# poja/Cattus

Hardware: AMD Instinct MI355X
Metric: MCTS node-evals/sec (chess 20x256 net, batch 256) (higher is better)
Workload: dtype f16x2

## Files before the change

### cattus_amd/csrc/evaluator.hip

```cpp
#include <hip/hip_runtime.h>

#include <algorithm>
#include <atomic>
#include <chrono>
#include <condition_variable>
#include <cmath>
#include <cstdarg>
#include <cstdio>
#include <cstdlib>
#include <cstring>
#include <deque>
#include <functional>
#include <map>
#include <memory>
#include <mutex>
#include <new>
#include <shared_mutex>
#include <string>
#include <thread>
#include <vector>

#include <dlfcn.h>

#include "../../include/cattus_hip.h"
// ... 102 lines not shown
    void* p = nullptr;
    bool owned = true;
    ~DevBuf() {
        if (p && owned) (void)hipFree(p);
    }
    int alloc(size_t bytes, DevArena* arena = nullptr) {
        if (p && owned) (void)hipFree(p);
        p = nullptr, owned = true;
        if (arena && (p = arena->take(bytes ? bytes : 16))) {
            owned = false;
            return CATTUS_OK;
        }
        hipError_t e = hipMalloc(&p, bytes ? bytes : 16);
        if (e != hipSuccess) return fail(CATTUS_E_NOMEM, "hipMalloc(%zu) failed: %s", bytes, hipGetErrorString(e));
        return CATTUS_OK;
    }
    int upload(const void* src, size_t bytes, DevArena* arena = nullptr) {
        int rc = alloc(bytes, arena);
        if (rc) return rc;
        HIP_TRY(hipMemcpy(p, src, bytes, hipMemcpyHostToDevice));
        return CATTUS_OK;
    }
    template <typename T>
    T* as() const {
        return reinterpret_cast<T*>(p);
    }
};

struct PinnedBuf {
    void* p = nullptr;
    ~PinnedBuf() {
        if (p) (void)hipHostFree(p);
    }
    int alloc(size_t bytes) {
        hipError_t e = hipHostMalloc(&p, bytes ? bytes : 16, hipHostMallocDefault);
        if (e != hipSuccess) return fail(CATTUS_E_NOMEM, "hipHostMalloc(%zu) failed: %s", bytes, hipGetErrorString(e));
        return CATTUS_OK;
    }
    template <typename T>
    T* as() const {
        return reinterpret_cast<T*>(p);
    }
};

std::shared_mutex g_pin_mu;
std::map<const char*, size_t> g_pinned;
struct Roctx {
    int (*push)(const char*) = nullptr;
    int (*pop)() = nullptr;
    Roctx() {
        const char* on = getenv("CATTUS_ROCTX");
        if (!on || on[0] != '1') return;
        for (const char* name : {"librocprofiler-sdk-roctx.so", "libroctx64.so"}) {
            if (void* h = dlopen(name, RTLD_NOW | RTLD_GLOBAL)) {
                push = reinterpret_cast<int (*)(const char*)>(dlsym(h, "roctxRangePushA"));
                pop = reinterpret_cast<int (*)()>(dlsym(h, "roctxRangePop"));
                if (push && pop) return;
                push = nullptr, pop = nullptr;
            }
        }
    }
};
const Roctx& roctx() {
    static const Roctx r;
    return r;
}
struct RoctxRange {
    bool on;
// ... 17 lines not shown
    return (const char*)p < it->first + it->second;
}

struct ConvLayer {
    DevBuf w, b;
    DevBuf wf;
    DevBuf wu, bw;
    uint32_t cin = 0;
};

struct ServerBatch {
    uint64_t seq = 0;
    uint32_t count = 0, collected = 0;
    bool sealed = false, running = false, done = false;
    int status = CATTUS_OK;
    std::string error;
    std::chrono::steady_clock::time_point t0;
    std::vector<uint64_t> planes;
    std::vector<float> policy, value;
    std::vector<uint8_t> taken;
};

constexpr int NLANES = CATTUS_HIP_LANES;

struct Lane {
    hipStream_t stream = nullptr;
    hipEvent_t done = nullptr;
    DevBuf d_planes, x0, a, t, y, hv, h1, d_policy, d_value;
    DevBuf d_legal_idx, d_legal_cnt, d_probs;
    uint32_t legal_stride = 0;
    PinnedBuf h_planes, h_policy, h_value;
    DevBuf tower_layers, tower_ready;
    PinnedBuf h_tower_err;
    uint32_t tower_nlayers = 0;
    std::mutex mu;
    ~Lane() {
        if (done) (void)hipEventDestroy(done);
        if (stream) (void)hipStreamDestroy(stream);
    }
};

}

struct cattus_eval {
    DevArena arena;
    cattus_net_desc d{};
    cattus_eval_config cfg{};
    bool tuned = false;
    bool simple = false;
    DevBuf d1w, d1b, d2w, d2b, svw, svb, spw, spb;
    bool wait_spin = true;
    Act act = Act::F32;
    uint32_t hw = 0, bpad = 0, cpad0 = 0;
    uint32_t slots = 64;
    uint32_t fpad = 0;
    bool tower64 = false;
    bool resident_tower = true;
    DevBuf t64_layers;
    bool tower64s = false;
    DevBuf t64s_bias;
    bool t64s_fuse_heads = true;
    int t64s_depth = 0;
    bool pack_separately = false;
    int t64_force_ch = 0;
    bool winograd = false;
    bool wino_k4 = true;
    bool wino_k8 = false;
    bool wino_persist = true;
    std::atomic<bool> persist_ok{true};
    uint32_t persist_spin = 1u << 18;
    uint32_t cus = 0;
    bool wino_inplace = true;
    bool split_wfrag = true;
    bool stream_shift_on = true;
    int stream_shift = 0;
    ConvOpts conv_opts;
    DevBuf d_saturated;
    bool t64_layer_steps = true;
    int device = 0;

    ConvLayer stem;
    std::vector<std::unique_ptr<ConvLayer>> c1, c2;
    DevBuf head_w, head_b, w1t, b1, w2, b2, wpt, bp;
    uint32_t kvp = 0, kpp = 0;

    Lane lanes[NLANES];
    std::atomic<unsigned> lane_rr{0};

    std::mutex stat_mu;
    cattus_stats stats{};
    uint64_t stats_tower_fallbacks = 0;

    std::mutex srv_mu;
    std::condition_variable srv_cv, done_cv;
    std::deque<std::unique_ptr<ServerBatch>> batches;
    uint64_t next_seq = 1;
    bool flush_req = false, stop = false;
    std::thread servers[NLANES];

    ~cattus_eval() {
        {
            std::lock_guard<std::mutex> lk(srv_mu);
            stop = true;
        }
        srv_cv.notify_all();
        done_cv.notify_all();
        for (auto& t : servers)
            if (t.joinable()) t.join();
    }
};

namespace {

size_t blob_floats(const cattus_net_desc& d) {
    const size_t hw = (size_t)d.board * d.board, F = d.filters;
    if (F == 0) {
        const size_t K = (size_t)d.planes * hw;
        return 2 * (K * K + K) + K + 1 + (size_t)d.moves * K + d.moves;
    }
    size_t n = F * d.planes * 9 + 4 * F;
    n += (size_t)d.blocks * (2 * F * F * 9 + 6 * F);
    n += (size_t)d.vhc * F + 2 * (size_t)d.vhc + (size_t)FC_HIDDEN * d.vhc * hw + FC_HIDDEN + FC_HIDDEN + 1;
    n += (size_t)d.phc * F + 2 * (size_t)d.phc + (size_t)d.moves * d.phc * hw + d.moves;
    return n;
}

bool wino_shape_ok(const cattus_eval* e, uint32_t cin, uint32_t cout) {
    return e->wino_k4 ? wino4_supported(e->bpad, cin, cout, e->d.board) : wino_supported(e->bpad, cin, cout, e->d.board);
}

std::mutex g_chain_mu;
hipEvent_t g_chain[64] = {};
int chain_persistent_launch(int device, hipStream_t st, const std::function<void()>& launch) {
    std::lock_guard<std::mutex> lk(g_chain_mu);
    hipEvent_t& ev = g_chain[device & 63];
    if (!ev) {
        HIP_TRY(hipEventCreateWithFlags(&ev, hipEventDisableTiming));
    } else {
        HIP_TRY(hipStreamWaitEvent(st, ev, 0));
    }
    launch();
    HIP_TRY(hipEventRecord(ev, st));
    return CATTUS_OK;
}

int upload_conv(cattus_eval* e, ConvLayer& L, const Folded& f, uint32_t cout, uint32_t cin, uint32_t cout_pad, uint32_t cin_pad) {
    int rc;
    if (!e->tuned) {
        L.cin = cin;
        if ((rc = L.b.upload(f.b.data(), cout * sizeof(float)))) return rc;
        return L.w.upload(f.w.data(), f.w.size() * sizeof(float));
    }
    L.cin = cin_pad;
    if (e->act == Act::F16S) {
        std::vector<float> b((size_t)2 * cout_pad, 0.0f);
        memcpy(b.data(), f.b.data(), cout * sizeof(float));
        std::vector<_Float16> w((size_t)9 * cout_pad * 2 * cin_pad, (_Float16)0.0f);
        for (uint32_t co = 0; co < cout_pad; co++) {
            float m = 0.0f;
            if (co < cout)
                for (uint32_t t = 0; t < 9; t++)
                    for (uint32_t ci = 0; ci < cin; ci++) m = std::max(m, fabsf(f.w[((size_t)t * cout + co) * cin + ci]));
            int sh = 0;
            if (m > 0.0f && std::isfinite(m)) sh = std::min(100, std::max(-100, 10 - ilogbf(m)));
            b[cout_pad + co] = ldexpf(1.0f, -sh);
            if (co >= cout) continue;
            for (uint32_t t = 0; t < 9; t++)
                for (uint32_t ci = 0; ci < cin; ci++) {
                    const float ws = ldexpf(f.w[((size_t)t * cout + co) * cin + ci], sh);
                    const _Float16 hi = (_Float16)ws;
                    const _Float16 lo = (_Float16)(ws - (float)hi);
                    _Float16* row = &w[((size_t)t * cout_pad + co) * 2 * cin_pad + (size_t)(ci >> 5) * 64 + (ci & 31)];
                    row[0] = hi, row[32] = lo;
                }
// ... 253 lines not shown
    }

    const size_t bp_ = e->bpad, B = e->cfg.max_batch;
    const size_t esz = e->tuned ? (act_f16_family(e->act) ? 4 : (size_t)act_bytes(e->act)) : 4;
    const size_t hesz = e->tuned ? (size_t)act_bytes(head_act(e->act)) : 4;
    const size_t slots = e->tuned ? e->slots : hw;
    const size_t FA = e->tuned ? FP : F;
    for (Lane& L : e->lanes) {
        HIP_TRY(hipStreamCreateWithFlags(&L.stream, hipStreamNonBlocking));
        HIP_TRY(hipEventCreateWithFlags(&L.done, hipEventBlockingSync | hipEventDisableTiming));
        if ((rc = L.d_planes.alloc(B * d.planes * e->cfg.plane_words * 8))) return rc;
        if ((rc = L.x0.alloc(bp_ * slots * e->cpad0 * esz))) return rc;
        if ((rc = L.a.alloc(bp_ * slots * FA * esz, &e->arena))) return rc;
        if ((rc = L.t.alloc(bp_ * slots * FA * esz, &e->arena))) return rc;
        if ((rc = L.y.alloc(bp_ * slots * FA * esz, e->wino_inplace ? nullptr : &e->arena))) return rc;
        const size_t hv_bytes = (size_t)(e->tuned ? (bp_ + 31) / 32 * 32 : bp_) * (e->kvp + e->kpp) * hesz;
        if ((rc = L.hv.alloc(hv_bytes))) return rc;
        HIP_TRY(hipMemset(L.hv.p, 0, hv_bytes));
        if ((rc = L.h1.alloc(bp_ * FC_HIDDEN * 4))) return rc;
        if ((rc = L.d_policy.alloc(B * d.moves * 4))) return rc;
        if ((rc = L.d_value.alloc(B * 4))) return rc;
        if ((rc = L.h_planes.alloc(B * d.planes * e->cfg.plane_words * 8))) return rc;
        if ((rc = L.h_policy.alloc(B * d.moves * 4))) return rc;
        if ((rc = L.h_value.alloc(B * 4))) return rc;
        if (e->tuned && e->act == Act::F16S && e->wino_k4 && e->wino_persist && e->wino_inplace && d.blocks > 0 && e->c1[0]->wu.p) {
            std::vector<Wino4TowerLayer> tl;
            for (uint32_t i = 0; i < d.blocks; i++) {
                tl.push_back(Wino4TowerLayer{L.a.as<float>(), e->c1[i]->wu.p, e->c1[i]->bw.as<float>(), nullptr, L.t.as<float>()});
                tl.push_back(Wino4TowerLayer{L.t.as<float>(), e->c2[i]->wu.p, e->c2[i]->bw.as<float>(), L.a.as<float>(), L.a.as<float>()});
            }
            L.tower_nlayers = (uint32_t)tl.size();
            if ((rc = L.tower_layers.upload(tl.data(), tl.size() * sizeof(Wino4TowerLayer)))) return rc;
            if ((rc = L.tower_ready.alloc(64 + (size_t)tl.size() * (bp_ / 4) * 4))) return rc;
            if ((rc = L.h_tower_err.alloc(4))) return rc;
            *L.h_tower_err.as<unsigned>() = 0;
        }
    }
    return CATTUS_OK;
}

struct TowerTimer {
    std::vector<hipEvent_t> ev;
    size_t used = 0;
};

int enqueue_forward(cattus_eval* e, Lane& L, const uint64_t* d_planes, uint32_t n, float* d_policy, float* d_value,
                    hipStream_t st, TowerTimer* tt = nullptr) {
    const cattus_net_desc& d = e->d;
    const uint32_t F = d.filters, hw = e->hw, S = d.board, w64 = e->cfg.plane_words;
    auto ev = [&](bool stop) -> hipEvent_t {
        if (!tt || tt->used >= tt->ev.size()) return nullptr;
        (void)stop;
        return tt->ev[tt->used++];
    };
    void *a = L.a.p, *t = L.t.p, *y = L.y.p;
    uint32_t nb = n;
    if (e->simple) {
        const uint32_t K = d.planes * hw;
        launch_planes_to_tensor_nchw(d_planes, n, d.planes, w64, S, n, L.x0.as<float>(), st);
        launch_dense(L.x0.as<float>(), K, e->d1w.as<float>(), e->d1b.as<float>(), n, K, K, (float*)a, 1, st);
        launch_dense((float*)a, K, e->d2w.as<float>(), e->d2b.as<float>(), n, K, K, (float*)t, 1, st);
        launch_dense((float*)t, K, e->svw.as<float>(), e->svb.as<float>(), n, K, 1, d_value, 2, st);
        launch_dense((float*)t, K, e->spw.as<float>(), e->spb.as<float>(), n, K, d.moves, d_policy, 0, st);
        hipError_t serr = hipGetLastError();
        if (serr != hipSuccess) return fail(CATTUS_E_DEVICE, "kernel launch failed: %s", hipGetErrorString(serr));
        return CATTUS_OK;
    }
    if (e->tuned) {
// ... 17 lines not shown
            ta.bias_all = e->t64s_bias.as<float>();
            ta.n = n, ta.C = d.planes, ta.w64 = w64, ta.S = S, ta.nlayers = 1 + 2 * d.blocks;
            if (e->t64s_fuse_heads) {
                ta.head_w = e->head_w.as<float>(), ta.head_b = e->head_b.as<float>(), ta.hv = L.hv.as<float>();
                ta.hv_pol = (uint32_t)((e->bpad + 31) / 32 * 32) * e->kvp, ta.kvp = e->kvp, ta.kpp = e->kpp, ta.vhc = d.vhc, ta.ocn = d.vhc + d.phc;
            } else {
                ta.out = (float*)a;
            }
            hipEvent_t s0 = ev(false), s1 = ev(true);
            launch_tower64_split(ta, nb * e->slots, e->t64s_depth, st, s0, s1);
        } else {
            const bool fused_stem = d.planes <= 32 && e->cpad0 == (uint32_t)act_kc(e->act) && !e->pack_separately;
            const StemInput stem_in{d_planes, n, d.planes, w64};
            if (!fused_stem) launch_pack_planes_nhwc(e->act, d_planes, n, nb, d.planes, w64, S, e->cpad0, L.x0.p, st);
            hipEvent_t s0 = ev(false), s1 = ev(true);
            const int last_flags = act_f16_family(e->act) ? CONV_OUT_F32 : 0;
            const bool wfrag = e->act == Act::F16S && e->split_wfrag;
            const int wflag = wfrag ? CONV_W_FRAG : 0;
            auto wptr = [&](const ConvLayer& c) { return wfrag ? c.wf.p : c.w.p; };
            launch_conv3x3_mfma(e->act, L.x0.p, wptr(e->stem), e->stem.b.as<float>(), nullptr, a, nb, e->cpad0, FP, S, st, s0, s1,
                                fused_stem ? &stem_in : nullptr,
                                wflag | (d.blocks == 0 ? last_flags : e->act == Act::F16S && e->c1[0]->wu.p ? CONV_OUT_F32 | CONV_WINO_IN : 0), e->conv_opts);
            const bool wino = d.blocks > 0 && e->c1[0]->wu.p != nullptr;
            auto conv = [&](const ConvLayer& c, const void* in, const void* res, void* out, int lflags) {
                hipEvent_t s0 = ev(false), s1 = ev(true);
                if (wino && e->wino_k8) launch_conv3x3_wino8((const float*)in, c.wu.p, c.bw.as<float>(), (const float*)res, (float*)out, nb, FP, FP, st, s0, s1, e->conv_opts.saturated);
                else if (wino && e->wino_k4) launch_conv3x3_wino4((const float*)in, c.wu.p, c.bw.as<float>(), (const float*)res, (float*)out, nb, FP, FP, st, s0, s1, e->conv_opts.saturated);
                else if (wino) launch_conv3x3_wino((const float*)in, c.wu.p, c.bw.as<float>(), (const float*)res, (float*)out, nb, FP, FP, st, s0, s1, e->conv_opts.saturated);
                else launch_conv3x3_mfma(e->act, in, wptr(c), c.b.as<float>(), res, out, nb, FP, FP, S, st, s0, s1, nullptr, wflag | lflags, e->conv_opts);
            };
            if (wino && !e->wino_k8 && L.tower_nlayers && e->persist_ok.load(std::memory_order_relaxed) && wino4_tower_fits(nb, FP, e->cus)) {
                hipEvent_t s0 = ev(false), s1 = ev(true);
                unsigned* const tower_err = L.tower_ready.as<unsigned>();
                HIP_TRY(hipMemsetAsync(L.tower_ready.p, 0, 64 + (size_t)L.tower_nlayers * (nb / 4) * 4, st));
                int crc = chain_persistent_launch(e->device, st, [&] {
                    launch_tower_wino4(L.tower_layers.as<Wino4TowerLayer>(), L.tower_nlayers, tower_err + 16, tower_err,
                                       e->conv_opts.saturated, nb, FP, e->persist_spin, e->cus, st, s0, s1);
                });
                if (crc) return crc;
                HIP_TRY(hipMemcpyAsync(L.h_tower_err.p, tower_err, 4, hipMemcpyDeviceToHost, st));
            } else
            for (uint32_t i = 0; i < d.blocks; i++) {
                conv(*e->c1[i], a, nullptr, t, 0);
                if (wino && e->wino_inplace) {
                    conv(*e->c2[i], t, a, a, 0);
                    continue;
                }
                conv(*e->c2[i], t, a, y, i + 1 == d.blocks ? last_flags : 0);
                std::swap(a, y);
            }
        }
    } else {
        launch_planes_to_tensor_nchw(d_planes, n, d.planes, w64, S, n, L.x0.as<float>(), st);
        hipEvent_t s0 = ev(false), s1 = ev(true);
        launch_conv3x3_generic(L.x0.as<float>(), e->stem.w.as<float>(), e->stem.b.as<float>(), nullptr, (float*)a, n,
                               d.planes, F, S, st, s0, s1);
        for (uint32_t i = 0; i < d.blocks; i++) {
            s0 = ev(false), s1 = ev(true);
            launch_conv3x3_generic((float*)a, e->c1[i]->w.as<float>(), e->c1[i]->b.as<float>(), nullptr, (float*)t, n, F,
                                   F, S, st, s0, s1);
            s0 = ev(false), s1 = ev(true);
            launch_conv3x3_generic((float*)t, e->c2[i]->w.as<float>(), e->c2[i]->b.as<float>(), (float*)a, (float*)y, n,
                                   F, F, S, st, s0, s1);
            std::swap(a, y);
        }
    }
    const uint32_t kv = d.vhc * hw, kp = d.phc * hw;
    if (e->tuned) {
        HeadsMfma hd{};
        hd.conv_w = e->head_w.p, hd.conv_b = e->head_b.as<float>(), hd.hv = L.hv.p;
        hd.w1 = e->w1t.p, hd.b1 = e->b1.as<float>(), hd.h1 = L.h1.as<float>();
        hd.wp = e->wpt.p, hd.bp = e->bp.as<float>(), hd.policy = d_policy;
        hd.hw = hw, hd.vhc = d.vhc, hd.phc = d.phc, hd.kvp = e->kvp, hd.kpp = e->kpp, hd.M = d.moves;
// ... 62 lines not shown
    }
    const void* src_planes = planes;
    if (!direct) {
        memcpy(L.h_planes.p, planes, pbytes);
        src_planes = L.h_planes.p;
    }
    HIP_TRY(hipMemcpyAsync(L.d_planes.p, src_planes, pbytes, hipMemcpyHostToDevice, L.stream));
    auto copy_out = [&]() -> int {
        if (lg) {
            HIP_TRY(hipMemcpyAsync(L.d_legal_idx.p, lg->idx, (size_t)n * lg->stride * 2, hipMemcpyHostToDevice, L.stream));
            HIP_TRY(hipMemcpyAsync(L.d_legal_cnt.p, lg->cnt, (size_t)n * 2, hipMemcpyHostToDevice, L.stream));
            if (launch_legal_softmax(L.d_policy.as<float>(), d.moves, L.d_legal_idx.as<uint16_t>(), L.d_legal_cnt.as<uint16_t>(),
                                     lg->stride, n, L.d_probs.as<float>(), L.stream))
                return fail(CATTUS_E_INVALID, "legal stride %u exceeds 1024", lg->stride);
            HIP_TRY(hipMemcpyAsync(lg->probs, L.d_probs.p, (size_t)n * lg->stride * 4, hipMemcpyDeviceToHost, L.stream));
        } else {
            HIP_TRY(hipMemcpyAsync(direct ? (void*)policy : L.h_policy.p, L.d_policy.p, (size_t)n * d.moves * 4, hipMemcpyDeviceToHost, L.stream));
        }
        HIP_TRY(hipMemcpyAsync(direct ? (void*)value : L.h_value.p, L.d_value.p, (size_t)n * 4, hipMemcpyDeviceToHost, L.stream));
        return CATTUS_OK;
    };
    auto run_batch = [&]() -> int {
        int rc = enqueue_forward(e, L, L.d_planes.as<uint64_t>(), n, L.d_policy.as<float>(), L.d_value.as<float>(), L.stream);
        if (rc) return rc;
        if ((rc = copy_out())) return rc;
        if (e->wait_spin) {
            HIP_TRY(hipStreamSynchronize(L.stream));
        } else {
            HIP_TRY(hipEventRecord(L.done, L.stream));
            HIP_TRY(hipEventSynchronize(L.done));
        }
        return CATTUS_OK;
    };
    int rc = run_batch();
    if (rc) return rc;
    if (L.h_tower_err.p && *L.h_tower_err.as<volatile unsigned>() != 0) {
        *L.h_tower_err.as<volatile unsigned>() = 0;
        e->persist_ok.store(false, std::memory_order_relaxed);
        {
            std::lock_guard<std::mutex> sl(e->stat_mu);
            e->stats_tower_fallbacks += 1;
        }
        if ((rc = run_batch())) return rc;
    }
    if (!direct) {
        if (!lg) memcpy(policy, L.h_policy.p, (size_t)n * d.moves * 4);
        memcpy(value, L.h_value.p, (size_t)n * 4);
    }
    account(e, n, std::chrono::duration<double>(std::chrono::steady_clock::now() - t0).count());
    return CATTUS_OK;
}

ServerBatch* new_batch(cattus_eval* e) {
    auto b = std::make_unique<ServerBatch>();
    b->seq = e->next_seq++;
    b->planes.resize((size_t)e->cfg.max_batch * e->d.planes * e->cfg.plane_words);
    e->batches.push_back(std::move(b));
    return e->batches.back().get();
}

void server_loop(cattus_eval* e) {
    std::unique_lock<std::mutex> lk(e->srv_mu);
    for (;;) {
        ServerBatch* run = nullptr;
        for (auto& b : e->batches)
            if (b->sealed && !b->done && !b->running) {
                run = b.get();
                break;
            }
        if (!run && !e->batches.empty()) {
// ... 28 lines not shown
        run->error = err;
        run->done = true;
        e->done_cv.notify_all();
    }
}

}


CATTUS_API const char* cattus_hip_last_error(void) { return g_last_error.c_str(); }
CATTUS_API const char* cattus_hip_version(void) { return "cattus_hip 0.2 (gfx950)"; }
CATTUS_API const char* cattus_hip_runtime_note(void) { return g_runtime_note.c_str(); }

CATTUS_API const char* cattus_hip_tower_kernel(const cattus_eval* e) {
    if (!e) return "";
    if (e->simple) return "policy_fc_kernel";
    if (!e->tuned) return "conv3x3_generic_kernel";
    if (e->tower64) return "tower64_lds_kernel";
    if (e->tower64s) return "tower64_split_kernel";
    if (e->act == Act::F16S) return e->d.blocks > 0 && e->c1[0]->wu.p ? (e->wino_k8 ? "conv3x3_wino8_kernel" : e->wino_k4 ? (e->lanes[0].tower_nlayers && e->persist_ok.load() && wino4_tower_fits(e->bpad, e->fpad, e->cus) ? "tower_wino4_kernel" : "conv3x3_wino4_kernel") : "conv3x3_wino_kernel") : e->split_wfrag ? "conv3x3_splitw_kernel" : "conv3x3_split_kernel";
    return "conv3x3_mfma_v2_kernel";
}

CATTUS_API int cattus_hip_stream_shift(const cattus_eval* e) { return e ? e->stream_shift : 0; }

namespace {

struct Switches {
    std::map<std::string, std::string> kv;
    int parse(const char* text) {
        if (!text) return CATTUS_OK;
        static const char* const known[] = {"CATTUS_CONV_CB", "CATTUS_CONV_PBW", "CATTUS_FUSED_STEM", "CATTUS_T64_CH", "CATTUS_T64_LS", "CATTUS_SPLIT_W",
                                            "CATTUS_T64S_HEADS", "CATTUS_T64S_SHAPE", "CATTUS_TOWER64", "CATTUS_FORCE_GENERIC", "CATTUS_WINO_INPLACE",
                                            "CATTUS_ARENA", "CATTUS_WINO_KERNEL", "CATTUS_WINO_PERSIST", "CATTUS_WINO_SPIN", "CATTUS_STREAM_SHIFT"};
        const std::string s(text);
        size_t at = 0;
        while (at < s.size()) {
            size_t end = s.find(';', at);
            if (end == std::string::npos) end = s.size();
            const std::string item = s.substr(at, end - at);
            at = end + 1;
            if (item.empty()) continue;
            const size_t eq = item.find('=');
            if (eq == std::string::npos || eq == 0) return fail(CATTUS_E_INVALID, "diagnostic switch '%s' is not KEY=VALUE", item.c_str());
            const std::string key = item.substr(0, eq);
            bool ok = false;
            for (const char* k : known) ok = ok || key == k;
            if (!ok) return fail(CATTUS_E_INVALID, "unknown diagnostic switch '%s'", key.c_str());
            kv[key] = item.substr(eq + 1);
        }
        return CATTUS_OK;
    }
    const char* get(const char* key) const {
        auto it = kv.find(key);
        return it == kv.end() ? nullptr : it->second.c_str();
    }
};

int create_impl(const void* weights, size_t nbytes, const cattus_eval_config* cfg_in, const char* switches, cattus_eval** out) {
    if (!out) return fail(CATTUS_E_INVALID, "out is NULL");
    *out = nullptr;
    if (!weights || !cfg_in) return fail(CATTUS_E_INVALID, "weights/cfg is NULL");
    cattus_eval_config cfg_copy{};
    if (cfg_in->struct_size == offsetof(cattus_eval_config, tower_form)) memcpy(&cfg_copy, cfg_in, offsetof(cattus_eval_config, tower_form));
    else if (cfg_in->struct_size == sizeof(cattus_eval_config)) cfg_copy = *cfg_in;
    else return fail(CATTUS_E_INVALID, "cfg.struct_size mismatch");
    cfg_copy.struct_size = sizeof(cattus_eval_config);
// ... 84 lines not shown
             : cfg->dtype == CATTUS_DTYPE_F16X2 ? Act::F16S
             : cfg->dtype == CATTUS_DTYPE_F16 ? Act::F16
                                              : Act::F32;
    if (!e->tuned && e->act != Act::F32)
        return fail(CATTUS_E_UNSUPPORTED, "bf16 / f16 / f16x2 need the MFMA tower: value + policy head channels <= 32 (got %u + %u)", d.vhc, d.phc);
    if (act_f16_family(e->act)) {
        int src = e->d_saturated.alloc(sizeof(unsigned));
        if (src) return src;
        HIP_TRY(hipMemset(e->d_saturated.p, 0, sizeof(unsigned)));
        e->conv_opts.saturated = e->d_saturated.as<unsigned>();
    }
    if (act_f16_family(e->act)) {
        if (d.planes > 32) return fail(CATTUS_E_UNSUPPORTED, "f16x2 / f16 take at most 32 input planes (got %u)", d.planes);
        e->pack_separately = false;
    }
    e->slots = tower_slots(d.board);
    e->fpad = e->tuned ? (d.filters + COUT_PER_WG - 1) / COUT_PER_WG * COUT_PER_WG : d.filters;
    const uint32_t bpw = e->tuned ? ROWS_PER_WG / e->slots : 1;
    e->bpad = (cfg->max_batch + bpw - 1) / bpw * bpw;
    const char* inplace_env = sw.get("CATTUS_WINO_INPLACE");
    e->wino_inplace = !(inplace_env && inplace_env[0] == '0');
    const char* arena_env = sw.get("CATTUS_ARENA");
    {
        const char* wk = sw.get("CATTUS_WINO_KERNEL");
        if (wk && strcmp(wk, "k16") != 0 && strcmp(wk, "k4") != 0 && strcmp(wk, "k8") != 0) return fail(CATTUS_E_INVALID, "CATTUS_WINO_KERNEL is k16, k4 or k8");
        e->wino_k8 = wk && strcmp(wk, "k8") == 0;
        e->wino_k4 = wk ? strcmp(wk, "k4") == 0 || e->wino_k8 : wino4_supported(e->bpad, e->fpad, e->fpad, d.board);
    }
    {
        const char* wp = sw.get("CATTUS_WINO_PERSIST");
        e->wino_persist = !(wp && wp[0] == '0');
        const char* ws = sw.get("CATTUS_WINO_SPIN");
        if (ws) e->persist_spin = (uint32_t)std::max(1L, atol(ws));
        hipDeviceProp_t prop;
        HIP_TRY(hipGetDeviceProperties(&prop, cfg->device));
        e->cus = (uint32_t)prop.multiProcessorCount;
    }
    if (cfg->tower_form == CATTUS_TOWER_WINOGRAD && !(e->tuned && e->act == Act::F16S && d.blocks > 0 && wino_shape_ok(e.get(), e->fpad, e->fpad)))
        return fail(CATTUS_E_UNSUPPORTED, "tower_form WINOGRAD needs dtype f16x2, an 8x8 board, at least one residual block and a multiple of 64 filters");
    if (e->tuned && e->act == Act::F16S && e->winograd && d.blocks > 0 && wino_shape_ok(e.get(), e->fpad, e->fpad) &&
        !(arena_env && arena_env[0] == '0')) {
        auto page = [](size_t b) { return (b + 4095) & ~(size_t)4095; };
        const size_t FPz = e->fpad, u_bytes = page(((size_t)16 * FPz * FPz * 2 + (size_t)WINO_RING_STAGES * 1024) * 2);
        const size_t act_bytes_ = page((size_t)e->bpad * e->slots * FPz * 4);
        const size_t want = 2 * (size_t)d.blocks * u_bytes + (size_t)NLANES * (e->wino_inplace ? 2 : 3) * act_bytes_ + (1u << 20);
        void* base = nullptr;
        if (hipMalloc(&base, want) == hipSuccess) e->arena.base = (char*)base, e->arena.cap = want;
        else (void)hipGetLastError();
    }
    int rc = build(e.get(), reinterpret_cast<const float*>((const char*)weights + HEADER_BYTES));
    if (rc) return rc;
    HIP_TRY(hipDeviceSynchronize());
    {
        std::lock_guard<std::mutex> lk(e->srv_mu);
        new_batch(e.get());
    }
    for (auto& t : e->servers) t = std::thread(server_loop, e.get());
    *out = e.release();
    return CATTUS_OK;
}

}

CATTUS_API int cattus_hip_create(const void* weights, size_t nbytes, const cattus_eval_config* cfg, cattus_eval** out) {
    return create_impl(weights, nbytes, cfg, nullptr, out);
}
// ... 14 lines not shown
    if (!e || !planes || !policy || !value) return fail(CATTUS_E_INVALID, "NULL argument");
    if (n < 1 || n > e->cfg.max_batch) return fail(CATTUS_E_INVALID, "invalid sample len %u, 1..=%u", n, e->cfg.max_batch);
    return eval_host(e, planes, n, policy, value);
}

CATTUS_API int cattus_hip_eval_legal(cattus_eval* e, const uint64_t* planes, uint32_t n, const uint16_t* legal_idx,
                                     const uint16_t* legal_count, uint32_t legal_stride, float* probs, float* value) {
    if (!e || !planes || !legal_idx || !legal_count || !probs || !value) return fail(CATTUS_E_INVALID, "NULL argument");
    if (n < 1 || n > e->cfg.max_batch) return fail(CATTUS_E_INVALID, "invalid sample len %u, 1..=%u", n, e->cfg.max_batch);
    if (legal_stride < 1 || legal_stride > 1024) return fail(CATTUS_E_INVALID, "legal_stride %u outside 1..=1024", legal_stride);
    for (uint32_t i = 0; i < n; i++) {
        if (legal_count[i] > legal_stride) return fail(CATTUS_E_INVALID, "leaf %u: %u legal moves > stride %u", i, legal_count[i], legal_stride);
        for (uint32_t k = 0; k < legal_count[i]; k++)
            if (legal_idx[(size_t)i * legal_stride + k] >= e->d.moves)
                return fail(CATTUS_E_INVALID, "leaf %u: policy index %u >= %u", i, legal_idx[(size_t)i * legal_stride + k], e->d.moves);
    }
    const LegalArgs lg{legal_idx, legal_count, legal_stride, probs};
    return eval_host(e, planes, n, nullptr, value, &lg);
}

CATTUS_API int cattus_hip_eval_device(cattus_eval* e, const uint64_t* d_planes, uint32_t n, float* d_policy, float* d_value,
                                      void* stream) {
    return cattus_hip_eval_device_lane(e, 0, d_planes, n, d_policy, d_value, stream);
}

CATTUS_API int cattus_hip_eval_device_lane(cattus_eval* e, uint32_t lane, const uint64_t* d_planes, uint32_t n, float* d_policy,
                                           float* d_value, void* stream) {
    if (!e || !d_planes || !d_policy || !d_value) return fail(CATTUS_E_INVALID, "NULL argument");
    if (n < 1 || n > e->cfg.max_batch) return fail(CATTUS_E_INVALID, "invalid sample len %u, 1..=%u", n, e->cfg.max_batch);
    if (lane >= NLANES) return fail(CATTUS_E_INVALID, "lane %u out of range (%d lanes)", lane, NLANES);
    Lane& L = e->lanes[lane];
    std::lock_guard<std::mutex> lk(L.mu);
    HIP_TRY(hipSetDevice(e->device));
    if (L.h_tower_err.p && *L.h_tower_err.as<volatile unsigned>() != 0) {
        *L.h_tower_err.as<volatile unsigned>() = 0;
        e->persist_ok.store(false, std::memory_order_relaxed);
        return fail(CATTUS_E_DEVICE, "an earlier batch on lane %u ran the tower as one launch and a hand-off wait in it gave up (the device was shared): that batch's "
                                     "outputs are invalid; this evaluator uses the per-layer launches from now on", lane);
    }
    hipStream_t st = (hipStream_t)stream;
    int rc = enqueue_forward(e, L, d_planes, n, d_policy, d_value, st);
    if (rc) return rc;
    std::lock_guard<std::mutex> sl(e->stat_mu);
    e->stats.batches += 1;
    e->stats.positions += n;
    if (n == e->cfg.max_batch) e->stats.full_batches += 1;
    return CATTUS_OK;
}

CATTUS_API int cattus_hip_lane_stream(cattus_eval* e, uint32_t lane, void** stream) {
    if (!e || !stream) return fail(CATTUS_E_INVALID, "NULL argument");
    if (lane >= NLANES) return fail(CATTUS_E_INVALID, "lane %u out of range (%d lanes)", lane, NLANES);
    *stream = (void*)e->lanes[lane].stream;
    return CATTUS_OK;
}

CATTUS_API int cattus_hip_submit(cattus_eval* e, const uint64_t* planes_one, uint64_t* ticket) {
    if (!e || !planes_one || !ticket) return fail(CATTUS_E_INVALID, "NULL argument");
    const size_t words = (size_t)e->d.planes * e->cfg.plane_words;
    std::unique_lock<std::mutex> lk(e->srv_mu);
    if (e->stop) return fail(CATTUS_E_STATE, "evaluator is shutting down");
    ServerBatch* cur = e->batches.empty() ? nullptr : e->batches.back().get();
    if (!cur || cur->sealed) cur = new_batch(e);
    const uint32_t slot = cur->count++;
    if (slot == 0) cur->t0 = std::chrono::steady_clock::now();
    memcpy(cur->planes.data() + slot * words, planes_one, words * 8);
    *ticket = (cur->seq << 32) | slot;
    const bool full = cur->count == e->cfg.max_batch;
    if (full) {
        cur->sealed = true;
        new_batch(e);
// ... 207 lines not shown
```

### cattus_amd/csrc/kernels.h

```cpp
#pragma once
#include <hip/hip_runtime.h>
#include <stdint.h>

namespace cattus {

inline uint32_t tower_slots(uint32_t S) { return S <= 8 ? 64u : 128u; }
constexpr int ROWS_PER_WG = 256;
constexpr int COUT_PER_WG = 64;

enum class Act : int { F32 = 0, BF16 = 1, F16S = 2, F16 = 3 };

inline bool act_two_bytes(Act a) { return a == Act::BF16 || a == Act::F16; }
inline int act_bytes(Act a) { return act_two_bytes(a) ? 2 : 4; }
inline int act_kc(Act a) { return act_two_bytes(a) ? 64 : 32; }
inline Act head_act(Act a) { return a == Act::BF16 ? Act::BF16 : Act::F32; }
inline bool act_f16_family(Act a) { return a == Act::F16S || a == Act::F16; }

hipError_t prepare_device();

void launch_pack_planes_nhwc(Act act, const uint64_t* planes, uint32_t n, uint32_t bpad, uint32_t C,
                             uint32_t w64, uint32_t S, uint32_t cpad, void* out, hipStream_t st);
void launch_planes_to_tensor_nchw(const uint64_t* planes, uint32_t n, uint32_t C, uint32_t w64, uint32_t S,
                                  uint32_t batch, float* out, hipStream_t st);

// ... 6 lines not shown
inline size_t split_frag_index(uint32_t t, uint32_t co, uint32_t ci, uint32_t part, uint32_t cin_pad) {
    const uint32_t nst = cin_pad / 32 * 18, ch = ci >> 5, k = (ci >> 4) & 1, h = (ci >> 3) & 1, e = ci & 7;
    const uint32_t stage = ((ch * 3 + t / 3) * 3 + t % 3) * 2 + k, lane = h * 32 + (co & 31);
    return ((((size_t)(co >> 5) * nst + stage) * 2 + part) * 64 + lane) * 8 + e;
}
struct ConvOpts {
    int cb = 0;
    int pbw = 0;
    unsigned* saturated = nullptr;
};
void launch_conv3x3_mfma(Act act, const void* in, const void* w, const float* bias, const void* res, void* out,
                         uint32_t bpad, uint32_t cin, uint32_t cout, uint32_t S, hipStream_t st,
                         hipEvent_t ev_start = nullptr, hipEvent_t ev_stop = nullptr, const StemInput* stem = nullptr,
                         int flags = 0, const ConvOpts& opts = ConvOpts());

constexpr int WINO_RING_STAGES = 8;
bool wino_supported(uint32_t bpad, uint32_t cin, uint32_t cout, uint32_t S);
inline size_t wino_frag_index(uint32_t f, uint32_t co, uint32_t ci, uint32_t part, uint32_t cin_pad) {
    const uint32_t nst = cin_pad / 16 * 16, stage = (ci >> 4) * 16 + f, lane = ((ci >> 3) & 1) * 32 + (co & 31);
    return ((((size_t)(co >> 5) * nst + stage) * 2 + part) * 64 + lane) * 8 + (ci & 7);
}
void launch_conv3x3_wino(const float* in, const void* wu, const float* bias, const float* res, float* out, uint32_t bpad, uint32_t cin,
                         uint32_t cout, hipStream_t st, hipEvent_t ev_start, hipEvent_t ev_stop, unsigned* sat);
hipError_t prepare_wino();

bool wino4_supported(uint32_t bpad, uint32_t cin, uint32_t cout, uint32_t S);
void launch_conv3x3_wino4(const float* in, const void* wu, const float* bias, const float* res, float* out, uint32_t bpad, uint32_t cin,
                          uint32_t cout, hipStream_t st, hipEvent_t ev_start, hipEvent_t ev_stop, unsigned* sat);
hipError_t prepare_wino4();
bool wino8_supported(uint32_t bpad, uint32_t cin, uint32_t cout, uint32_t S);
void launch_conv3x3_wino8(const float* in, const void* wu, const float* bias, const float* res, float* out, uint32_t bpad, uint32_t cin,
                          uint32_t cout, hipStream_t st, hipEvent_t ev_start, hipEvent_t ev_stop, unsigned* sat);
hipError_t prepare_wino8();
struct Wino4TowerLayer {
    const float* in;
    const void* wu;
    const float* bias;
    const float* res;
    float* out;
};
bool wino4_tower_fits(uint32_t bpad, uint32_t filters, uint32_t cus);
void launch_tower_wino4(const Wino4TowerLayer* d_layers, uint32_t nlayers, unsigned* ready, unsigned* err, unsigned* sat, uint32_t bpad, uint32_t filters,
                        uint32_t spin_budget, uint32_t cus, hipStream_t st, hipEvent_t ev_start, hipEvent_t ev_stop);

double launch_mfma_sustain(Act act, int cus, int iters, float* out, hipStream_t st);

struct Tower64Layer {
    const void* w;
    const float* bias;
    int res;
    int pad_;
};
struct Tower64Args {
    const uint64_t* planes;
    const Tower64Layer* layers;
    void* out;
    uint32_t n, C, w64, S, nlayers;
    const void* head_w;
    const float* head_b;
    void* hv;
    uint32_t hv_pol, kvp, kpp, vhc, ocn;
};
void launch_tower64(const Tower64Args& args, uint32_t rows, int ch, bool layer_steps, hipStream_t st,
                    hipEvent_t ev_start = nullptr, hipEvent_t ev_stop = nullptr);

struct Tower64SplitLayer {
    const void* wf;
    const float* bias;
    int res;
    int nch;
};
struct Tower64SplitArgs {
    const uint64_t* planes;
    const Tower64SplitLayer* layers;
    const float* bias_all;
    float* out;
// ... 54 lines not shown
```

### cattus_amd/csrc/kernels_wino4.hip

```cpp
#include "kernels.h"
#include "device_common.h"

#include <hip/hip_ext.h>

namespace cattus {

constexpr int W4_TROW = 8 * SP;
constexpr int W4_IMG = 9472;
constexpr int W4_ZAREA = 512;
constexpr int W4_IMGZ = W4_IMG + W4_ZAREA;
constexpr int W4_DBUF = 8 * W4_IMGZ;
constexpr int W4_LDS_LOOP = 2 * W4_DBUF;
constexpr int W4_LDS_Z = 4 * 2 * 64 * 256;
constexpr int W4_LDS_TOTAL = W4_LDS_Z > W4_LDS_LOOP ? W4_LDS_Z : W4_LDS_LOOP;
static_assert(W4_IMG % 256 == 0 && W4_IMGZ % 256 == 0 && W4_DBUF % 256 == 0, "the zero area keeps a read's banks only if everything is 256-B aligned");
static_assert(W4_IMG >= 8 * W4_TROW + 16 && W4_ZAREA >= 256 + 128 && W4_LDS_LOOP <= 160 * 1024, "image / zero area / LDS sizes");

typedef __attribute__((ext_vector_type(2))) _Float16 w4_f16x2;

template <int V>
using w4_int = std::integral_constant<int, V>;

#ifdef CATTUS_STAMPS
__device__ unsigned long long g_stamps_w4[1024 * 4 * 10];
#define W4_STAMP(i) st_[i] = __builtin_amdgcn_s_memtime()
#define W4_STAMP_RT(i) st_[i] = __builtin_amdgcn_s_memrealtime()
#else
#define W4_STAMP(i)
#define W4_STAMP_RT(i)
#endif

struct W4Sync {
    const unsigned* wait_word;
    unsigned* done_word;
    unsigned* err;
    unsigned wait_target;
    unsigned spin_budget;
};

template <int RES, bool PERSIST>
__device__ __forceinline__ void w4_layer(const float* __restrict__ in, const _Float16* __restrict__ wu, const float* __restrict__ bias,
                                         const float* res, float* out, unsigned* __restrict__ sat, int cin, int cout, char* smem,
                                         const W4Sync& sync, int wg, int nblk) {
    typedef _Float16 T;
    typedef Mfma<T>::frag frag;
    constexpr bool has_res = RES == 1;

#ifdef CATTUS_STAMPS
    unsigned long long st_[10] = {0, 0, 0, 0, 0, 0, 0, 0, 0, 0};
#endif
    W4_STAMP(0);
    W4_STAMP_RT(6);
    int tid = threadIdx.x;
    asm volatile("" : "+v"(tid));
    const int q = __builtin_amdgcn_readfirstlane(tid >> 6);
    const int lane = tid & 63;

    const int ncg = cout >> 6;
    int logical = wg;
    if ((nblk & 7) == 0) logical = (wg & 7) * (nblk >> 3) + (wg >> 3);
    const int cout0 = (logical % ncg) * 64;
    const int row0 = (logical / ncg) * 256;

    const int nch = cin >> 5;
    const int nks = cin >> 4;
    const uint32_t row_bytes = (uint32_t)cin * 4;

    const char* wb0 = reinterpret_cast<const char*>(wu) + ((size_t)(cout0 >> 5) * nks * 16 + 4 * q) * SW_STAGE;
// ... 32 lines not shown
#pragma unroll
        for (int i = 0; i < W4_NP; i++) load_piece(regs[i], ch, i);
    };
    auto t_unit = [&](const u32x4(&regs)[W4_NP], uint32_t target, int u) __attribute__((always_inline)) {
        const int fq = u >> 2, ty = u & 3;
        const int ra = fq == 0 ? 0 : fq == 2 ? 2 : 1, rb = fq == 3 ? 3 : fq == 2 ? 1 : 2;
        const int ya = 2 * ty - 1 + ra, yb = 2 * ty - 1 + rb;
        u32x4 t;
        if (yb > 7) t = regs[ya];
        else {
#pragma unroll
            for (int e = 0; e < 4; e++) {
                if (ya < 0) asm("v_fma_f32 %0, %1, -1.0, 0" : "=v"(t[e]) : "v"(regs[yb][e]));
                else if (fq == 1) asm("v_fma_f32 %0, %1, 1.0, %2" : "=v"(t[e]) : "v"(regs[yb][e]), "v"(regs[ya][e]));
                else asm("v_fma_f32 %0, %1, -1.0, %2" : "=v"(t[e]) : "v"(regs[yb][e]), "v"(regs[ya][e]));
            }
        }
        typedef __attribute__((address_space(3))) u32x4 w4_lu32x4;
        *(w4_lu32x4*)(uintptr_t)(target + (uint32_t)(fq * 2 * W4_IMGZ + ty * W4_TROW)) = t;
    };
    for (int i = tid; i < 16 * (W4_ZAREA / 16); i += 256)
        reinterpret_cast<f32x4*>(smem + (i / (W4_ZAREA / 16)) * W4_IMGZ + W4_IMG)[i % (W4_ZAREA / 16)] = f32x4{0.f, 0.f, 0.f, 0.f};
    u32x4 first[W4_NP], pend[W4_NP];
    const char* wks = wb0;
    load_ustage(ring[0], wks, 0);
    load_ustage(ring[1], wks, 1);
    if (PERSIST && sync.wait_word) {
        if (tid == 0) {
            unsigned budget = sync.spin_budget, seen = 0, bad = 0;
            for (;;) {
                asm volatile("global_load_dword %0, %1, off sc1\n\ts_waitcnt vmcnt(0)" : "=v"(seen) : "v"(sync.wait_word) : "memory");
                if (seen >= sync.wait_target) break;
                if ((budget & 63) == 0) asm volatile("global_load_dword %0, %1, off sc1\n\ts_waitcnt vmcnt(0)" : "=v"(bad) : "v"(sync.err) : "memory");
                if (bad != 0 || --budget == 0) {
                    atomicExch(sync.err, 1u);
                    break;
                }
                __builtin_amdgcn_s_sleep(8);
            }
        }
        asm volatile("s_barrier" ::: "memory");
    }
    W4_STAMP(8);
    load_chunk(first, 0);
    load_chunk(pend, 1);
    load_ustage(ring[2], wks, 2);

    const int n = lane & 31, hh = lane >> 5;
    const int b2 = n >> 4, ty = (n >> 2) & 3, tx = n & 3;
    uint32_t cur[3];
    {
        const int tbase = (b2 * 4 + ty) * W4_TROW + (2 * tx - 1) * SP + b2 * 16 + hh * 32;
        const int tdelta = tbase - W4_IMG;
        const int mc0 = tx != 0 ? -1 : 255, mc3 = tx != 3 ? -1 : 255;
        const uint32_t img = lds0 + (uint32_t)(q * 2 * W4_IMGZ + W4_IMG);
        cur[0] = img + (uint32_t)(tdelta & mc0);
        cur[1] = img + (uint32_t)(tdelta + SP);
        cur[2] = img + (uint32_t)(((tdelta + 3 * SP) & mc3));
    }
    int bufstep = W4_DBUF;

    u32x4 vh01[2][2], vl01[2][2], vh23[2][2][2], vl23[2][2][2];
    f32x4 tbuf[2][4];
    f32x4 xx;
    float vmax = 0.0f;

    auto freq_slot = [&](int sp, int tbv, int g, int l, int half) __attribute__((always_inline)) {
        if (half == 0) {
// ... 210 lines not shown
            v[j] = x < WINO_ACT_MAX ? x : WINO_ACT_MAX;
        }
        vmax = fmaxf(fmaxf(vmax, fmaxf(v[0], v[1])), fmaxf(v[2], v[3]));
        if (PERSIST) asm volatile("global_store_dwordx4 %0, %1, %2 sc1\n\ts_nop 1" ::"v"(evoff + k * cstride), "v"(v), "s"(obase) : "memory");
        else *reinterpret_cast<f32x4*>(out + (orow + k) * (size_t)cout + cout0 + pc * 4) = v;
    }
    if (vmax >= WINO_ACT_MAX) atomicAdd(sat, 1u);
    if (PERSIST) {
        asm volatile("s_waitcnt vmcnt(0)" ::: "memory");
        W4_STAMP(9);
        asm volatile("s_barrier" ::: "memory");
        if (tid == 0) __hip_atomic_fetch_add(sync.done_word, 1u, __ATOMIC_RELAXED, __HIP_MEMORY_SCOPE_AGENT);
    }
#ifdef CATTUS_STAMPS
    W4_STAMP(5);
    W4_STAMP_RT(7);
    if (lane == 0 && blockIdx.x < 1024) {
#pragma unroll
        for (int i = 0; i < 10; i++) g_stamps_w4[((size_t)blockIdx.x * 4 + q) * 10 + i] = st_[i];
    }
#endif
}

template <bool HAS_RES>
__global__ void __launch_bounds__(256, 1)
    conv3x3_wino4_kernel(const float* __restrict__ in, const _Float16* __restrict__ wu, const float* __restrict__ bias,
                         const float* res, float* out, unsigned* __restrict__ sat, int cin, int cout) {
    extern __shared__ __attribute__((aligned(16))) char smem[];
    const W4Sync none{};
    w4_layer<HAS_RES ? 1 : 0, false>(in, wu, bias, res, out, sat, cin, cout, smem, none, (int)blockIdx.x, (int)gridDim.x);
}

__global__ void __launch_bounds__(256, 1)
    tower_wino4_kernel(const Wino4TowerLayer* __restrict__ layers, int nlayers, unsigned* ready, unsigned* err, unsigned* __restrict__ sat, int filters,
                       unsigned spin_budget, int tiles) {
    extern __shared__ __attribute__((aligned(16))) char smem[];
    const int ncg = filters >> 6, ngroups = tiles / ncg;
    auto group_of = [&](int wg) {
        int logical = wg;
        if ((tiles & 7) == 0) logical = (wg & 7) * (tiles >> 3) + (wg >> 3);
        return logical / ncg;
    };
    auto sync_of = [&](int layer, int group) {
        W4Sync sync;
        sync.wait_word = layer > 0 ? ready + (size_t)(layer - 1) * ngroups + group : nullptr;
        sync.done_word = ready + (size_t)layer * ngroups + group;
        sync.err = err, sync.wait_target = (unsigned)ncg, sync.spin_budget = spin_budget;
        return sync;
    };
    for (int layer = 0; layer + 1 < nlayers; layer += 2) {
        const Wino4TowerLayer A = layers[layer];
        for (int wg = blockIdx.x; wg < tiles; wg += gridDim.x)
            w4_layer<0, true>(A.in, reinterpret_cast<const _Float16*>(A.wu), A.bias, nullptr, A.out, sat, filters, filters, smem, sync_of(layer, group_of(wg)), wg, tiles);
        const Wino4TowerLayer B = layers[layer + 1];
        for (int wg = blockIdx.x; wg < tiles; wg += gridDim.x)
            w4_layer<1, true>(B.in, reinterpret_cast<const _Float16*>(B.wu), B.bias, B.res, B.out, sat, filters, filters, smem, sync_of(layer + 1, group_of(wg)), wg, tiles);
    }
}

bool wino4_supported(uint32_t bpad, uint32_t cin, uint32_t cout, uint32_t S) {
    return S == 8 && cin >= 128 && cin % 32 == 0 && cout >= 128 && cout % 64 == 0 && bpad % 4 == 0;
}

void launch_conv3x3_wino4(const float* in, const void* wu, const float* bias, const float* res, float* out, uint32_t bpad, uint32_t cin,
                          uint32_t cout, hipStream_t st, hipEvent_t ev_start, hipEvent_t ev_stop, unsigned* sat) {
    typedef _Float16 H;
    const dim3 grid((bpad / 4) * (cout / 64));
    if (res)
        hipExtLaunchKernelGGL((conv3x3_wino4_kernel<true>), grid, dim3(256), W4_LDS_TOTAL, st, ev_start, ev_stop, 0, in, (const H*)wu, bias, res, out,
                              sat, (int)cin, (int)cout);
    else
        hipExtLaunchKernelGGL((conv3x3_wino4_kernel<false>), grid, dim3(256), W4_LDS_TOTAL, st, ev_start, ev_stop, 0, in, (const H*)wu, bias, res, out,
                              sat, (int)cin, (int)cout);
}

static uint32_t tower_grid(uint32_t tiles, uint32_t cus) { return tiles <= cus ? tiles : cus & ~7u; }

bool wino4_tower_fits(uint32_t bpad, uint32_t filters, uint32_t cus) {
    const uint32_t tiles = (bpad / 4) * (filters / 64);
    return tiles <= cus || (cus >= 8 && tiles % 8 == 0);
}

void launch_tower_wino4(const Wino4TowerLayer* d_layers, uint32_t nlayers, unsigned* ready, unsigned* err, unsigned* sat, uint32_t bpad, uint32_t filters,
                        uint32_t spin_budget, uint32_t cus, hipStream_t st, hipEvent_t ev_start, hipEvent_t ev_stop) {
    const uint32_t tiles = (bpad / 4) * (filters / 64);
    hipExtLaunchKernelGGL(tower_wino4_kernel, dim3(tower_grid(tiles, cus)), dim3(256), W4_LDS_TOTAL, st, ev_start, ev_stop, 0, d_layers, (int)nlayers, ready, err,
                          sat, (int)filters, spin_budget, (int)tiles);
}

#ifdef CATTUS_STAMPS
extern "C" __attribute__((visibility("default"))) int cattus_hip_debug_stamps_w4(unsigned long long* out, size_t n) {
    return (int)hipMemcpyFromSymbol(out, HIP_SYMBOL(g_stamps_w4), n * sizeof(unsigned long long));
}
#endif

hipError_t prepare_wino4() {
    hipError_t err = hipFuncSetAttribute(reinterpret_cast<const void*>(&conv3x3_wino4_kernel<true>), hipFuncAttributeMaxDynamicSharedMemorySize, W4_LDS_TOTAL);
    const hipError_t e2 = hipFuncSetAttribute(reinterpret_cast<const void*>(&conv3x3_wino4_kernel<false>), hipFuncAttributeMaxDynamicSharedMemorySize, W4_LDS_TOTAL);
    const hipError_t e3 = hipFuncSetAttribute(reinterpret_cast<const void*>(&tower_wino4_kernel), hipFuncAttributeMaxDynamicSharedMemorySize, W4_LDS_TOTAL);
    return err != hipSuccess ? err : e2 != hipSuccess ? e2 : e3;
}

}
```

Baseline: 216,200.

## Use epoch-based ready counters to drop per-batch memset and error readback

The persistent one-launch tower no longer clears its ready/error flags with a memset before every batch, and no longer copies the error word back to the host afterwards. Each launch gets an increasing epoch, and layer hand-off waits target epoch*ncg, so counters just keep growing. The host resets them only on epoch overflow or when the batch grows. Errors are now written straight by the kernel to mapped coherent host memory, tagged with a per-lane launch serial. The ready array is also re-laid out as group-major so each group's per-layer counters are contiguous. This removes two small stream operations per batch, at the cost of more complex error-attribution logic.

```diff
diff --git a/cattus_amd/csrc/evaluator.hip b/cattus_amd/csrc/evaluator.hip
--- a/cattus_amd/csrc/evaluator.hip
+++ b/cattus_amd/csrc/evaluator.hip
@@ -158,8 +158,8 @@
     ~PinnedBuf() {
         if (p) (void)hipHostFree(p);
     }
-    int alloc(size_t bytes) {
-        hipError_t e = hipHostMalloc(&p, bytes ? bytes : 16, hipHostMallocDefault);
+    int alloc(size_t bytes, unsigned flags = hipHostMallocDefault) {
+        hipError_t e = hipHostMalloc(&p, bytes ? bytes : 16, flags);
         if (e != hipSuccess) return fail(CATTUS_E_NOMEM, "hipHostMalloc(%zu) failed: %s", bytes, hipGetErrorString(e));
         return CATTUS_OK;
     }
@@ -243,7 +243,11 @@
     PinnedBuf h_planes, h_policy, h_value;
     DevBuf tower_layers, tower_ready;
     PinnedBuf h_tower_err;
+    W4HostErr* d_tower_err = nullptr;
     uint32_t tower_nlayers = 0;
+    uint64_t tower_serial = 0, tower_reported = 0, tower_host_handled = 0;
+    uint64_t tower_batch_serial = 0;
+    uint32_t tower_epoch = 0, tower_groups = 0;
     std::mutex mu;
     ~Lane() {
         if (done) (void)hipEventDestroy(done);
@@ -280,6 +284,7 @@
     bool wino_persist = true;
     std::atomic<bool> persist_ok{true};
     uint32_t persist_spin = 1u << 18;
+    uint32_t persist_max_epoch = 0;
     uint32_t cus = 0;
     bool wino_inplace = true;
     bool split_wfrag = true;
@@ -342,7 +347,7 @@
 
 std::mutex g_chain_mu;
 hipEvent_t g_chain[64] = {};
-int chain_persistent_launch(int device, hipStream_t st, const std::function<void()>& launch) {
+int chain_persistent_launch(int device, hipStream_t st, const std::function<int()>& launch) {
     std::lock_guard<std::mutex> lk(g_chain_mu);
     hipEvent_t& ev = g_chain[device & 63];
     if (!ev) {
@@ -350,7 +355,7 @@
     } else {
         HIP_TRY(hipStreamWaitEvent(st, ev, 0));
     }
-    launch();
+    if (int rc = launch()) return rc;
     HIP_TRY(hipEventRecord(ev, st));
     return CATTUS_OK;
 }
@@ -670,8 +675,11 @@
             L.tower_nlayers = (uint32_t)tl.size();
             if ((rc = L.tower_layers.upload(tl.data(), tl.size() * sizeof(Wino4TowerLayer)))) return rc;
             if ((rc = L.tower_ready.alloc(64 + (size_t)tl.size() * (bp_ / 4) * 4))) return rc;
-            if ((rc = L.h_tower_err.alloc(4))) return rc;
-            *L.h_tower_err.as<unsigned>() = 0;
+            HIP_TRY(hipMemset(L.tower_ready.p, 0, 64 + (size_t)tl.size() * (bp_ / 4) * 4));
+            L.tower_epoch = 0, L.tower_groups = (uint32_t)(bp_ / 4);
+            if ((rc = L.h_tower_err.alloc(sizeof(W4HostErr), hipHostMallocMapped | hipHostMallocCoherent))) return rc;
+            *L.h_tower_err.as<W4HostErr>() = W4HostErr{0, 0};
+            HIP_TRY(hipHostGetDevicePointer(reinterpret_cast<void**>(&L.d_tower_err), L.h_tower_err.p, 0));
         }
     }
     return CATTUS_OK;
@@ -755,13 +763,21 @@
             if (wino && !e->wino_k8 && L.tower_nlayers && e->persist_ok.load(std::memory_order_relaxed) && wino4_tower_fits(nb, FP, e->cus)) {
                 hipEvent_t s0 = ev(false), s1 = ev(true);
                 unsigned* const tower_err = L.tower_ready.as<unsigned>();
-                HIP_TRY(hipMemsetAsync(L.tower_ready.p, 0, 64 + (size_t)L.tower_nlayers * (nb / 4) * 4, st));
-                int crc = chain_persistent_launch(e->device, st, [&] {
-                    launch_tower_wino4(L.tower_layers.as<Wino4TowerLayer>(), L.tower_nlayers, tower_err + 16, tower_err,
+                const uint32_t groups = nb / 4;
+                int crc = chain_persistent_launch(e->device, st, [&]() -> int {
+                    if (L.tower_epoch >= e->persist_max_epoch || groups > L.tower_groups) {
+                        HIP_TRY(hipMemsetAsync(L.tower_ready.p, 0, 64 + (size_t)L.tower_nlayers * (e->bpad / 4) * 4, st));
+                        L.tower_epoch = 0, L.tower_groups = groups;
+                    }
+                    L.tower_epoch += 1;
+                    L.tower_groups = std::min(L.tower_groups, groups);
+                    L.tower_batch_serial = ++L.tower_serial;
+                    launch_tower_wino4(L.tower_layers.as<Wino4TowerLayer>(), L.tower_nlayers, tower_err + 16, tower_err, L.d_tower_err, L.tower_serial,
+                                       L.tower_reported, L.tower_epoch,
                                        e->conv_opts.saturated, nb, FP, e->persist_spin, e->cus, st, s0, s1);
+                    return CATTUS_OK;
                 });
                 if (crc) return crc;
-                HIP_TRY(hipMemcpyAsync(L.h_tower_err.p, tower_err, 4, hipMemcpyDeviceToHost, st));
             } else
             for (uint32_t i = 0; i < d.blocks; i++) {
                 conv(*e->c1[i], a, nullptr, t, 0);
@@ -890,10 +906,13 @@
         }
         return CATTUS_OK;
     };
+    L.tower_batch_serial = 0;
     int rc = run_batch();
     if (rc) return rc;
-    if (L.h_tower_err.p && *L.h_tower_err.as<volatile unsigned>() != 0) {
-        *L.h_tower_err.as<volatile unsigned>() = 0;
+    const uint64_t mine = L.tower_batch_serial;
+    if (mine != 0 && __atomic_load_n(&L.h_tower_err.as<W4HostErr>()->last, __ATOMIC_ACQUIRE) == mine) {
+        L.tower_host_handled = mine;
+        if (__atomic_load_n(&L.h_tower_err.as<W4HostErr>()->first, __ATOMIC_ACQUIRE) == mine) L.tower_reported = mine;
         e->persist_ok.store(false, std::memory_order_relaxed);
         {
             std::lock_guard<std::mutex> sl(e->stat_mu);
@@ -988,7 +1007,8 @@
         if (!text) return CATTUS_OK;
         static const char* const known[] = {"CATTUS_CONV_CB", "CATTUS_CONV_PBW", "CATTUS_FUSED_STEM", "CATTUS_T64_CH", "CATTUS_T64_LS", "CATTUS_SPLIT_W",
                                             "CATTUS_T64S_HEADS", "CATTUS_T64S_SHAPE", "CATTUS_TOWER64", "CATTUS_FORCE_GENERIC", "CATTUS_WINO_INPLACE",
-                                            "CATTUS_ARENA", "CATTUS_WINO_KERNEL", "CATTUS_WINO_PERSIST", "CATTUS_WINO_SPIN", "CATTUS_STREAM_SHIFT"};
+                                            "CATTUS_ARENA", "CATTUS_WINO_KERNEL", "CATTUS_WINO_PERSIST", "CATTUS_WINO_SPIN", "CATTUS_WINO_EPOCHS",
+                                            "CATTUS_STREAM_SHIFT"};
         const std::string s(text);
         size_t at = 0;
         while (at < s.size()) {
@@ -1139,6 +1159,9 @@
         e->wino_persist = !(wp && wp[0] == '0');
         const char* ws = sw.get("CATTUS_WINO_SPIN");
         if (ws) e->persist_spin = (uint32_t)std::max(1L, atol(ws));
+        e->persist_max_epoch = wino4_tower_max_epoch(e->fpad);
+        const char* we = sw.get("CATTUS_WINO_EPOCHS");
+        if (we) e->persist_max_epoch = std::min(e->persist_max_epoch, (uint32_t)std::max(1L, atol(we)));
         hipDeviceProp_t prop;
         HIP_TRY(hipGetDeviceProperties(&prop, cfg->device));
         e->cus = (uint32_t)prop.multiProcessorCount;
@@ -1219,11 +1242,17 @@
     Lane& L = e->lanes[lane];
     std::lock_guard<std::mutex> lk(L.mu);
     HIP_TRY(hipSetDevice(e->device));
-    if (L.h_tower_err.p && *L.h_tower_err.as<volatile unsigned>() != 0) {
-        *L.h_tower_err.as<volatile unsigned>() = 0;
-        e->persist_ok.store(false, std::memory_order_relaxed);
-        return fail(CATTUS_E_DEVICE, "an earlier batch on lane %u ran the tower as one launch and a hand-off wait in it gave up (the device was shared): that batch's "
-                                     "outputs are invalid; this evaluator uses the per-layer launches from now on", lane);
+    if (L.h_tower_err.p) {
+        const W4HostErr* he = L.h_tower_err.as<W4HostErr>();
+        const uint64_t first = __atomic_load_n(&he->first, __ATOMIC_ACQUIRE), last = __atomic_load_n(&he->last, __ATOMIC_ACQUIRE);
+        const uint64_t gave_up = first > L.tower_reported ? first : last > L.tower_reported && last != L.tower_host_handled ? last : 0;
+        if (gave_up) {
+            L.tower_reported = std::max(first, last);
+            e->persist_ok.store(false, std::memory_order_relaxed);
+            return fail(CATTUS_E_DEVICE, "an earlier batch on lane %u (one-launch tower launch %llu of the lane) ran the tower as one launch and a hand-off wait in it "
+                                         "gave up (the device was shared): that batch's outputs are invalid; this evaluator uses the per-layer launches from now on",
+                        lane, (unsigned long long)gave_up);
+        }
     }
     hipStream_t st = (hipStream_t)stream;
     int rc = enqueue_forward(e, L, d_planes, n, d_policy, d_value, st);
diff --git a/cattus_amd/csrc/kernels.h b/cattus_amd/csrc/kernels.h
--- a/cattus_amd/csrc/kernels.h
+++ b/cattus_amd/csrc/kernels.h
@@ -62,6 +62,9 @@
 void launch_conv3x3_wino8(const float* in, const void* wu, const float* bias, const float* res, float* out, uint32_t bpad, uint32_t cin,
                           uint32_t cout, hipStream_t st, hipEvent_t ev_start, hipEvent_t ev_stop, unsigned* sat);
 hipError_t prepare_wino8();
+struct W4HostErr {
+    unsigned long long first, last;
+};
 struct Wino4TowerLayer {
     const float* in;
     const void* wu;
@@ -70,8 +73,10 @@
     float* out;
 };
 bool wino4_tower_fits(uint32_t bpad, uint32_t filters, uint32_t cus);
-void launch_tower_wino4(const Wino4TowerLayer* d_layers, uint32_t nlayers, unsigned* ready, unsigned* err, unsigned* sat, uint32_t bpad, uint32_t filters,
-                        uint32_t spin_budget, uint32_t cus, hipStream_t st, hipEvent_t ev_start, hipEvent_t ev_stop);
+uint32_t wino4_tower_max_epoch(uint32_t filters);
+void launch_tower_wino4(const Wino4TowerLayer* d_layers, uint32_t nlayers, unsigned* ready, unsigned* err, W4HostErr* host_err, uint64_t serial,
+                        uint64_t reported, uint32_t epoch, unsigned* sat, uint32_t bpad, uint32_t filters, uint32_t spin_budget, uint32_t cus,
+                        hipStream_t st, hipEvent_t ev_start, hipEvent_t ev_stop);
 
 double launch_mfma_sustain(Act act, int cus, int iters, float* out, hipStream_t st);
 
diff --git a/cattus_amd/csrc/kernels_wino4.hip b/cattus_amd/csrc/kernels_wino4.hip
--- a/cattus_amd/csrc/kernels_wino4.hip
+++ b/cattus_amd/csrc/kernels_wino4.hip
@@ -34,6 +34,10 @@
     const unsigned* wait_word;
     unsigned* done_word;
     unsigned* err;
+    W4HostErr* host_err;
+    unsigned long long serial;
+    unsigned long long reported;
+    unsigned epoch;
     unsigned wait_target;
     unsigned spin_budget;
 };
@@ -132,8 +136,11 @@
                 asm volatile("global_load_dword %0, %1, off sc1\n\ts_waitcnt vmcnt(0)" : "=v"(seen) : "v"(sync.wait_word) : "memory");
                 if (seen >= sync.wait_target) break;
                 if ((budget & 63) == 0) asm volatile("global_load_dword %0, %1, off sc1\n\ts_waitcnt vmcnt(0)" : "=v"(bad) : "v"(sync.err) : "memory");
-                if (bad != 0 || --budget == 0) {
-                    atomicExch(sync.err, 1u);
+                if (bad == sync.epoch || --budget == 0) {
+                    atomicExch(sync.err, sync.epoch);
+                    if (__hip_atomic_load(&sync.host_err->first, __ATOMIC_RELAXED, __HIP_MEMORY_SCOPE_SYSTEM) <= sync.reported)
+                        __hip_atomic_store(&sync.host_err->first, sync.serial, __ATOMIC_RELAXED, __HIP_MEMORY_SCOPE_SYSTEM);
+                    __hip_atomic_store(&sync.host_err->last, sync.serial, __ATOMIC_RELAXED, __HIP_MEMORY_SCOPE_SYSTEM);
                     break;
                 }
                 __builtin_amdgcn_s_sleep(8);
@@ -410,10 +417,11 @@
 }
 
 __global__ void __launch_bounds__(256, 1)
-    tower_wino4_kernel(const Wino4TowerLayer* __restrict__ layers, int nlayers, unsigned* ready, unsigned* err, unsigned* __restrict__ sat, int filters,
+    tower_wino4_kernel(const Wino4TowerLayer* __restrict__ layers, int nlayers, unsigned* ready, unsigned* err, W4HostErr* host_err,
+                       unsigned long long serial, unsigned long long reported, unsigned epoch, unsigned* __restrict__ sat, int filters,
                        unsigned spin_budget, int tiles) {
     extern __shared__ __attribute__((aligned(16))) char smem[];
-    const int ncg = filters >> 6, ngroups = tiles / ncg;
+    const int ncg = filters >> 6;
     auto group_of = [&](int wg) {
         int logical = wg;
         if ((tiles & 7) == 0) logical = (wg & 7) * (tiles >> 3) + (wg >> 3);
@@ -421,9 +429,11 @@
     };
     auto sync_of = [&](int layer, int group) {
         W4Sync sync;
-        sync.wait_word = layer > 0 ? ready + (size_t)(layer - 1) * ngroups + group : nullptr;
-        sync.done_word = ready + (size_t)layer * ngroups + group;
-        sync.err = err, sync.wait_target = (unsigned)ncg, sync.spin_budget = spin_budget;
+        sync.wait_word = layer > 0 ? ready + (size_t)group * nlayers + layer - 1 : nullptr;
+        sync.done_word = ready + (size_t)group * nlayers + layer;
+        sync.err = err, sync.host_err = host_err, sync.serial = serial, sync.reported = reported;
+        sync.epoch = epoch, sync.spin_budget = spin_budget;
+        sync.wait_target = epoch * (unsigned)ncg;
         return sync;
     };
     for (int layer = 0; layer + 1 < nlayers; layer += 2) {
@@ -459,11 +469,14 @@
     return tiles <= cus || (cus >= 8 && tiles % 8 == 0);
 }
 
-void launch_tower_wino4(const Wino4TowerLayer* d_layers, uint32_t nlayers, unsigned* ready, unsigned* err, unsigned* sat, uint32_t bpad, uint32_t filters,
-                        uint32_t spin_budget, uint32_t cus, hipStream_t st, hipEvent_t ev_start, hipEvent_t ev_stop) {
+uint32_t wino4_tower_max_epoch(uint32_t filters) { return 0xFFFFFFFFu / (filters >= 64 ? filters / 64 : 1u); }
+
+void launch_tower_wino4(const Wino4TowerLayer* d_layers, uint32_t nlayers, unsigned* ready, unsigned* err, W4HostErr* host_err, uint64_t serial,
+                        uint64_t reported, uint32_t epoch, unsigned* sat, uint32_t bpad, uint32_t filters, uint32_t spin_budget, uint32_t cus,
+                        hipStream_t st, hipEvent_t ev_start, hipEvent_t ev_stop) {
     const uint32_t tiles = (bpad / 4) * (filters / 64);
     hipExtLaunchKernelGGL(tower_wino4_kernel, dim3(tower_grid(tiles, cus)), dim3(256), W4_LDS_TOTAL, st, ev_start, ev_stop, 0, d_layers, (int)nlayers, ready, err,
-                          sat, (int)filters, spin_budget, (int)tiles);
+                          host_err, (unsigned long long)serial, (unsigned long long)reported, epoch, sat, (int)filters, spin_budget, (int)tiles);
 }
 
 #ifdef CATTUS_STAMPS
```

Result: faster. 218,400, median of 6 (+1.0%).
